# liyi14/mx-DeepIM

Hardware: NVIDIA H100
Metric: 480x640 4-iter pose refinements/sec (higher is better)
Workload: dtype fp16

## Files before the change

mx-deepim_b200/csrc/conv_igemm.cuh:

```cuda
#pragma once
#include <cuda.h>
#include <cuda_fp16.h>
#include "common.cuh"
#include "wgmma.cuh"

namespace dim {

struct ConvKParams {
  CUtensorMap a_map[4];
  CUtensorMap a_lo_map[4];
  CUtensorMap b_map;
  CUtensorMap b_lo_map;
  CUtensorMap out_map[2];
  const __nv_bfloat16 *in_hi, *in_lo;
  int in_cols;
  int KH, KW, stride, cchunks;
  int BW, BH, n_col_tiles;
  int Hq, Ho, Wo, Bn;
  int out_Hp, out_Wp, out_py, out_px, Cout;
  int kblocks;
  float slope;
  const float *bias;
  __nv_bfloat16 *out_hi, *out_lo;
  int in_off_r, in_off_c;
// ... 46 lines not shown
  do {
    asm volatile(
        "{\n\t.reg .pred p;\n\tmbarrier.try_wait.parity.shared::cta.b64 p, [%1], %2;\n\tselp.u32 %0, 1, 0, p;\n\t}"
        : "=r"(ok)
        : "r"(addr), "r"(parity)
        : "memory");
  } while (!ok);
}
__device__ __forceinline__ void prefetch_tmap(const CUtensorMap *m) {
  asm volatile("prefetch.tensormap [%0];" ::"l"((uint64_t)m) : "memory");
}
__device__ __forceinline__ void tma_load_2d(void *dst, const CUtensorMap *map, uint64_t *bar, int c0, int c1) {
  if (elect_one())
    asm volatile(
        "cp.async.bulk.tensor.2d.shared::cluster.global.mbarrier::complete_tx::bytes [%0], [%1, {%3, %4}], [%2];" ::"r"(
            smem_u32(dst)),
        "l"((uint64_t)map), "r"(smem_u32(bar)), "r"(c0), "r"(c1)
        : "memory");
}
__device__ __forceinline__ void tma_load_3d(void *dst, const CUtensorMap *map, uint64_t *bar, int c0, int c1, int c2) {
  if (elect_one())
    asm volatile(
        "cp.async.bulk.tensor.3d.shared::cluster.global.mbarrier::complete_tx::bytes [%0], [%1, {%3, %4, %5}], [%2];" ::
            "r"(smem_u32(dst)),
        "l"((uint64_t)map), "r"(smem_u32(bar)), "r"(c0), "r"(c1), "r"(c2)
        : "memory");
}

__device__ __forceinline__ void mbar_arrive(uint64_t *bar) {
  asm volatile("mbarrier.arrive.shared::cta.b64 _, [%0];" ::"r"(smem_u32(bar)) : "memory");
}

__device__ __forceinline__ void bulk_load_raw(void *dst, const void *src, uint32_t bytes, uint64_t *bar) {
  asm volatile("cp.async.bulk.shared::cluster.global.mbarrier::complete_tx::bytes [%0], [%1], %2, [%3];" ::"r"(smem_u32(dst)),
               "l"(src), "r"(bytes), "r"(smem_u32(bar))
               : "memory");
}
__device__ __forceinline__ void tma_store_4d(const CUtensorMap *map, const void *src, int c0, int c1, int c2, int c3) {
  asm volatile("cp.async.bulk.tensor.4d.global.shared::cta.bulk_group [%0, {%2, %3, %4, %5}], [%1];" ::"l"((uint64_t)map),
               "r"(smem_u32(src)), "r"(c0), "r"(c1), "r"(c2), "r"(c3)
               : "memory");
}
__device__ __forceinline__ void bulk_commit() { asm volatile("cp.async.bulk.commit_group;" ::: "memory"); }
__device__ __forceinline__ void bulk_wait_read0() { asm volatile("cp.async.bulk.wait_group.read 0;" ::: "memory"); }
__device__ __forceinline__ void bulk_wait0() { asm volatile("cp.async.bulk.wait_group 0;" ::: "memory"); }
__device__ __forceinline__ void named_bar_sync(int id, int threads) {
  asm volatile("bar.sync %0, %1;" ::"r"(id), "r"(threads) : "memory");
}
__device__ __forceinline__ void stmatrix_x4_trans(uint32_t addr, const uint32_t (&r)[4]) {
  asm volatile("stmatrix.sync.aligned.m8n8.x4.trans.shared.b16 [%0], {%1, %2, %3, %4};" ::"r"(addr), "r"(r[0]), "r"(r[1]),
               "r"(r[2]), "r"(r[3])
               : "memory");
}

__device__ __forceinline__ void tma_load_4d(void *dst, const CUtensorMap *map, uint64_t *bar, int c0, int c1, int c2, int c3) {
  if (elect_one())
    asm volatile(
        "cp.async.bulk.tensor.4d.shared::cluster.global.mbarrier::complete_tx::bytes [%0], [%1, {%3, %4, %5, %6}], [%2];" ::
            "r"(smem_u32(dst)),
        "l"((uint64_t)map), "r"(smem_u32(bar)), "r"(c0), "r"(c1), "r"(c2), "r"(c3)
        : "memory");
}

__device__ __forceinline__ uint64_t gmma_desc(uint32_t saddr, uint32_t lbo_bytes, uint32_t sbo_bytes, uint32_t layout) {
  uint64_t d = 0;
  d |= (uint64_t)((saddr & 0x3FFFFu) >> 4);
  d |= (uint64_t)((lbo_bytes >> 4) & 0x3FFFu) << 16;
  d |= (uint64_t)((sbo_bytes >> 4) & 0x3FFFu) << 32;
  d |= (uint64_t)layout << 62;
  return d;
}
constexpr uint32_t kSW128 = 1u, kSW64 = 2u, kNoSwizzle = 0u;

__device__ __forceinline__ void regs_producer() { asm volatile("setmaxnreg.dec.sync.aligned.u32 40;"); }
__device__ __forceinline__ void regs_consumer() { asm volatile("setmaxnreg.inc.sync.aligned.u32 232;"); }

}

__device__ __forceinline__ uint32_t pack2_f16(float a, float b) {
  uint32_t r;
  asm("cvt.rn.satfinite.f16x2.f32 %0, %1, %2;" : "=r"(r) : "f"(b), "f"(a));
  return r;
}
__device__ __forceinline__ uint32_t pack2_bf16(float a, float b) {
  uint32_t r;
  asm("cvt.rn.bf16x2.f32 %0, %1, %2;" : "=r"(r) : "f"(b), "f"(a));
  return r;
}

constexpr int kConv1Slack = 2048;


__device__ __forceinline__ int frag_row(int t) { return ((t >> 5) << 4) + ((t & 31) >> 2); }

__device__ __forceinline__ uint32_t pack2_bf16_lo(float v0, float v1, uint32_t hi) {
  return pack2_bf16(v0 - __uint_as_float(hi << 16), v1 - __uint_as_float(hi & 0xFFFF0000u));
}

template <bool SPLIT3, bool F16>
__device__ __forceinline__ void epi_pack(float v0, float v1, float b0, float b1, float slope, uint32_t &hi, uint32_t &lo) {
  v0 += b0;
  v1 += b1;
  v0 = v0 > 0.f ? v0 : v0 * slope;
  v1 = v1 > 0.f ? v1 : v1 * slope;
  if (F16) {
    hi = pack2_f16(v0, v1);
  } else {
    hi = pack2_bf16(v0, v1);
    if (SPLIT3) lo = pack2_bf16_lo(v0, v1, hi);
  }
}

template <bool SPLIT3, bool F16>
__device__ __forceinline__ void store_pair(float v0, float v1, float2 b, float slope, __nv_bfloat16 *out_hi, __nv_bfloat16 *out_lo,
                                           long long off) {
  uint32_t h, l = 0;
  epi_pack<SPLIT3, F16>(v0, v1, b.x, b.y, slope, h, l);
  *reinterpret_cast<uint32_t *>(out_hi + off) = h;
  if (SPLIT3) *reinterpret_cast<uint32_t *>(out_lo + off) = l;
}

template <bool SPLIT3>
__device__ __forceinline__ void store_pair_generic(float v0, float v1, const ConvKParams &p, int n, bool valid, long long off,
                                                   long long add_off, long long mask_off) {
  if (!valid || n >= p.Cout) return;
  if (p.bias) {
    v0 += __ldg(p.bias + n);
    v1 += __ldg(p.bias + n + 1);
  }
  if (p.addend.p) {
    const __nv_bfloat162 a = *reinterpret_cast<const __nv_bfloat162 *>(p.addend.p + add_off);
    if (SPLIT3) {
      const __nv_bfloat162 al = *reinterpret_cast<const __nv_bfloat162 *>(p.addend.lo + add_off);
      v0 += __low2float(a) + __low2float(al);
      v1 += __high2float(a) + __high2float(al);
    } else {
      v0 += __low2float(a);
      v1 += __high2float(a);
    }
  }
  if (p.mask.p) {
    if (n < p.mask_climit) {
      const __nv_bfloat162 m = *reinterpret_cast<const __nv_bfloat162 *>(p.mask.p + mask_off);
      if (!(__low2float(m) > 0.f)) v0 *= p.slope;
      if (!(__high2float(m) > 0.f)) v1 *= p.slope;
    }
  } else {
    v0 = v0 > 0.f ? v0 : v0 * p.slope;
    v1 = v1 > 0.f ? v1 : v1 * p.slope;
  }
  if (SPLIT3) {
    const uint32_t h = pack2_bf16(v0, v1);
    *reinterpret_cast<uint32_t *>(p.out_hi + off) = h;
    *reinterpret_cast<uint32_t *>(p.out_lo + off) = pack2_bf16_lo(v0, v1, h);
  } else {
    *reinterpret_cast<__nv_bfloat162 *>(p.out_hi + off) = __floats2bfloat162_rn(v0, v1);
  }
}

template <int BLOCK_N, int STAGES, bool SPLIT3>
struct ConvSmem2 {
  static constexpr int A_BYTES = 128 * 64 * 2;
  static constexpr int B_BYTES = BLOCK_N * 64 * 2;
  static constexpr int NPREC = SPLIT3 ? 2 : 1;
  static constexpr int STAGE_BYTES = (A_BYTES + B_BYTES) * NPREC;
  static constexpr int TOTAL = STAGES * STAGE_BYTES + 1024  + 256 ;
  static_assert(TOTAL <= 227 * 1024, "conv_igemm shared memory");
};

template <int BLOCK_N, int STAGES, bool SPLIT3, bool F16, int EPI = 0>
__global__ void __launch_bounds__(384, 1) conv_igemm_persistent_kernel(const __grid_constant__ ConvKParams p,
                                                                       const int total_tiles, const int n_tiles) {
  using S = ConvSmem2<BLOCK_N, STAGES, SPLIT3>;
  constexpr uint32_t SBO = 1024u;

  extern __shared__ uint8_t smem_raw[];
  uint8_t *smem = reinterpret_cast<uint8_t *>((reinterpret_cast<uintptr_t>(smem_raw) + 1023) & ~(uintptr_t)1023);
  uint64_t *full_bar = reinterpret_cast<uint64_t *>(smem + STAGES * S::STAGE_BYTES);
  uint64_t *empty_bar = full_bar + STAGES;

  const int wgi = threadIdx.x >> 7, warp = threadIdx.x >> 5;

  if (threadIdx.x == 0) {
    for (int s = 0; s < STAGES; ++s) {
      ptx::mbar_init(&full_bar[s], 1);
      ptx::mbar_init(&empty_bar[s], 2);
    }
    ptx::fence_barrier_init();
    ptx::prefetch_tmap(&p.b_map);
    ptx::prefetch_tmap(&p.a_map[0]);
  }
  __syncthreads();

  if (wgi == 0) {
    ptx::regs_producer();
    if (warp == 0) {
      const uint32_t tx = (uint32_t)(p.BW * p.BH * 64 * 2 + BLOCK_N * 64 * 2) * S::NPREC;
      int s = 0;
      uint32_t ph = 0;
      for (int tile = blockIdx.x; tile < total_tiles; tile += gridDim.x) {
        const int nt = tile % n_tiles, mt = tile / n_tiles;
        const int col_tile = mt % p.n_col_tiles, row_tile = mt / p.n_col_tiles;
        const int g0 = row_tile * p.BH, ow0 = col_tile * p.BW, n0 = nt * BLOCK_N;
        for (int kb = 0; kb < p.kblocks; ++kb) {
          ptx::mbar_wait(&empty_bar[s], ph ^ 1u);
          const int tap = kb / p.cchunks, cc = kb - tap * p.cchunks;
          const int kh = tap / p.KW, kw = tap - kh * p.KW;
          int view = 0, dr = kh, dc = kw;
          if (p.stride == 2) {
            view = ((kh & 1) << 1) | (kw & 1);
            dr = kh >> 1;
            dc = kw >> 1;
          }
          uint8_t *st = smem + s * S::STAGE_BYTES;
          if (EPI) { dr += p.in_off_r; dc += p.in_off_c; }
          if (ptx::elect_one()) {
            ptx::mbar_expect_tx_raw(&full_bar[s], tx);
            ptx::tma_load_3d_raw(st, &p.a_map[view], &full_bar[s], cc * 64, ow0 + dc, g0 + dr);
            ptx::tma_load_2d_raw(st + S::A_BYTES, &p.b_map, &full_bar[s], kb * 64, n0);
            if (SPLIT3) {
              ptx::tma_load_3d_raw(st + S::A_BYTES + S::B_BYTES, &p.a_lo_map[view], &full_bar[s], cc * 64, ow0 + dc, g0 + dr);
              ptx::tma_load_2d_raw(st + 2 * S::A_BYTES + S::B_BYTES, &p.b_lo_map, &full_bar[s], kb * 64, n0);
            }
          }
          __syncwarp();
          if (++s == STAGES) { s = 0; ph ^= 1u; }
        }
      }
    }
  } else {
    ptx::regs_consumer();
    const int t = threadIdx.x & 127;
    const int half = wgi - 1;
    const int r0 = half * 64 + frag_row(t), q2 = (t & 3) * 2;
    const bool arriver = t == 0;
    const uint32_t base = ptx::smem_u32(smem);
    float acc[BLOCK_N / 2];
    int s = 0;
    uint32_t ph = 0;
    for (int tile = blockIdx.x; tile < total_tiles; tile += gridDim.x) {
      int prev = -1;
      for (int kb = 0; kb < p.kblocks; ++kb) {
        ptx::mbar_wait(&full_bar[s], ph);
        const uint32_t a_hi = base + s * S::STAGE_BYTES + half * 8192;
        const uint32_t b_hi = base + s * S::STAGE_BYTES + S::A_BYTES;
        const uint64_t da0 = ptx::gmma_desc(a_hi, 16, SBO, ptx::kSW128), db0 = ptx::gmma_desc(b_hi, 16, SBO, ptx::kSW128);
        const uint64_t dal0 = da0 + ((S::A_BYTES + S::B_BYTES) >> 4), dbl0 = db0 + ((S::A_BYTES + S::B_BYTES) >> 4);
        wg::fence_acc(acc);
        wg::fence();
#pragma unroll
        for (int k = 0; k < 4; ++k) {
          const uint64_t da = da0 + (uint64_t)(2 * k), db = db0 + (uint64_t)(2 * k);
          wg::mma<BLOCK_N, F16, 0, 0>(acc, da, db, (kb > 0 || k > 0) ? 1u : 0u);
          if (SPLIT3) {
            wg::mma<BLOCK_N, false, 0, 0>(acc, dal0 + (uint64_t)(2 * k), db, 1u);
            wg::mma<BLOCK_N, false, 0, 0>(acc, da, dbl0 + (uint64_t)(2 * k), 1u);
          }
        }
        wg::commit();
        wg::wait<1>();
        wg::fence_acc(acc);
        if (prev >= 0 && arriver) ptx::mbar_arrive(&empty_bar[prev]);
        prev = s;
        if (++s == STAGES) { s = 0; ph ^= 1u; }
      }
      wg::wait<0>();
      wg::fence_acc(acc);
      if (prev >= 0 && arriver) ptx::mbar_arrive(&empty_bar[prev]);

      const int nt = tile % n_tiles, mt = tile / n_tiles;
      const int col_tile = mt % p.n_col_tiles, row_tile = mt / p.n_col_tiles;
      const int n0 = nt * BLOCK_N;
#pragma unroll
      for (int rr = 0; rr < 2; ++rr) {
        const int m = r0 + rr * 8;
        const int bh = m / p.BW, bw = m - bh * p.BW;
        const int g = row_tile * p.BH + bh, ow = col_tile * p.BW + bw;
        const int n_img = g / p.Hq, oh = g - n_img * p.Hq;
        if (EPI == 1) {
          const int y = oh * p.out_sy + p.out_oy, x = ow * p.out_sx + p.out_ox;
          const bool valid = (m < p.BW * p.BH) && (n_img < p.Bn) && (oh < p.Ho) && (ow < p.Wo) && y >= 0 && y < p.out_H &&
                             x >= 0 && x < p.out_W;
          const long long off =
              (((long long)n_img * p.out_Hp + y + p.out_py) * p.out_Wp + x + p.out_px) * p.out_cs + p.out_coff + n0 + q2;
          const long long add_off =
              (((long long)n_img * p.addend.Hp + y + p.addend.py) * p.addend.Wp + x + p.addend.px) * p.addend.cs + p.addend.coff +
              n0 + q2;
          const long long mask_off =
              (((long long)n_img * p.mask.Hp + y + p.mask.py) * p.mask.Wp + x + p.mask.px) * p.mask.cs + p.mask.coff + n0 + q2;
#pragma unroll
          for (int j = 0; j < BLOCK_N / 8; ++j)
            store_pair_generic<SPLIT3>(acc[4 * j + 2 * rr], acc[4 * j + 2 * rr + 1], p, n0 + 8 * j + q2, valid, off + 8 * j,
                               add_off + 8 * j, mask_off + 8 * j);
        } else {
          const bool valid = (m < p.BW * p.BH) && (n_img < p.Bn) && (oh < p.Ho) && (ow < p.Wo);
          if (valid) {
            const long long off = (((long long)n_img * p.out_Hp + oh + p.out_py) * p.out_Wp + ow + p.out_px) * p.Cout + n0 + q2;
#pragma unroll
            for (int j = 0; j < BLOCK_N / 8; ++j)
              store_pair<SPLIT3, F16>(acc[4 * j + 2 * rr], acc[4 * j + 2 * rr + 1],
                                      make_float2(__ldg(p.bias + n0 + 8 * j + q2), __ldg(p.bias + n0 + 8 * j + q2 + 1)), p.slope, p.out_hi,
                                      p.out_lo, off + 8 * j);
          }
        }
      }
    }
  }
}

constexpr int kConv1StoreN = 80;

template <int N, int STAGES, bool SPLIT3>
struct Conv1Smem {
  static constexpr int NPREC = SPLIT3 ? 2 : 1;
  static constexpr int TAP_BYTES = 64 * 32 * 2;
  static constexpr int RES_BYTES = 16 * TAP_BYTES * NPREC;
  static constexpr int STG_BYTES = N * 128;
  static constexpr int PLANE_BYTES = (N + 3) * 16;
  static constexpr int STRIP_BYTES = (4 * PLANE_BYTES + 127) / 128 * 128;
  static constexpr int STAGE_BYTES = STRIP_BYTES * NPREC;
  static constexpr int TOTAL = RES_BYTES + 2 * STG_BYTES * NPREC + STAGES * STAGE_BYTES + 1024  + 256 ;
  static_assert(N % kConv1StoreN == 0 && N % 16 == 0 && STG_BYTES % 1024 == 0, "conv1 tile width");
  static_assert(TOTAL <= 227 * 1024, "conv1 shared memory");
};

template <int N, int STAGES, bool SPLIT3, bool F16>
__global__ void __launch_bounds__(384, 1) conv1_kernel(const __grid_constant__ ConvKParams p, const int rows_total,
                                                       const int rows_per_chunk, const int chunks_per_col) {
  using S = Conv1Smem<N, STAGES, SPLIT3>;
  extern __shared__ uint8_t smem_raw[];
  uint8_t *smem = reinterpret_cast<uint8_t *>((reinterpret_cast<uintptr_t>(smem_raw) + 1023) & ~(uintptr_t)1023);
  uint8_t *res = smem;
  uint8_t *stg = res + S::RES_BYTES;
  uint8_t *ring = stg + 2 * S::NPREC * S::STG_BYTES;
  uint64_t *full_bar = reinterpret_cast<uint64_t *>(ring + STAGES * S::STAGE_BYTES);
  uint64_t *empty_bar = full_bar + STAGES;
  uint64_t *res_bar = empty_bar + STAGES;

  const int wgi = threadIdx.x >> 7, warp = threadIdx.x >> 5;
  const int ct = blockIdx.x / chunks_per_col, ck = blockIdx.x - ct * chunks_per_col;
  const int g_lo = ck * rows_per_chunk;
  const int g_hi = min(rows_total, g_lo + rows_per_chunk);
  const int n_rows = max(0, g_hi - g_lo);
  const int n_strips = n_rows > 0 ? n_rows + 3 : 0;
  const int ow0 = ct * N;

  if (threadIdx.x == 0) {
    for (int s = 0; s < STAGES; ++s) {
      ptx::mbar_init(&full_bar[s], 1);
      ptx::mbar_init(&empty_bar[s], 2);
    }
    ptx::mbar_init(res_bar, 1);
    ptx::fence_barrier_init();
    ptx::prefetch_tmap(&p.b_map);
    ptx::prefetch_tmap(&p.out_map[0]);
  }
  __syncthreads();

  if (wgi == 0) {
// ... 260 lines not shown
```

mx-deepim_b200/csrc/net.cu:

```cuda
#include <cuda_fp16.h>
#include <string.h>

#include <memory>
#include <mutex>

#include "launch.cuh"
#include "net_state.cuh"

namespace dim {

static void build_geometry(NetState *ns, int H, int W) {
  int h = H, w = W;
  for (int i = 0; i < 10; ++i) {
    const LayerSpec &s = kLayers[i];
    LayerGeom &g = ns->g[i];
    g.Cin = s.Cin; g.Cout = s.Cout; g.k = s.k; g.stride = s.stride; g.pad = s.pad;
    g.Hin = h; g.Win = w;
    g.Ho = (h + 2 * s.pad - s.k) / s.stride + 1;
    g.Wo = (w + 2 * s.pad - s.k) / s.stride + 1;
    if (g.Ho < 1) g.Ho = 1;
    if (g.Wo < 1) g.Wo = 1;
    int Hp = h + 2 * s.pad, Wp = w + 2 * s.pad;
    if (s.stride == 2) { Hp += Hp & 1; Wp += Wp & 1; }
    g.py = g.px = s.pad;
// ... 26 lines not shown
    if (i == 0) {
      const int nt = cdiv(g.Wo, 128);
      g.BW = cdiv(g.Wo, nt); g.BH = 1; g.n_col_tiles = nt;
    }
    g.kblocks = g.KH * g.KW * (g.Ceff / g.BLOCK_K);
    h = g.Ho; w = g.Wo;
  }
}

typedef CUresult (*EncodeTiledFn)(CUtensorMap *, CUtensorMapDataType, cuuint32_t, void *, const cuuint64_t *,
                                  const cuuint64_t *, const cuuint32_t *, const cuuint32_t *, CUtensorMapInterleave,
                                  CUtensorMapSwizzle, CUtensorMapL2promotion, CUtensorMapFloatOOBfill);
static EncodeTiledFn get_encode() {
  static EncodeTiledFn fn = nullptr;
  if (!fn) {
    void *p = nullptr;
    cudaDriverEntryPointQueryResult q;
    if (cudaGetDriverEntryPoint("cuTensorMapEncodeTiled", &p, cudaEnableDefault, &q) == cudaSuccess &&
        q == cudaDriverEntryPointSuccess)
      fn = reinterpret_cast<EncodeTiledFn>(p);
  }
  return fn;
}

int encode_map(CUtensorMap *m, void *base, int rank, const uint64_t *dims, const uint64_t *strides_bytes,
                      const uint32_t *box, int block_k ) {
  EncodeTiledFn fn = get_encode();
  DIM_REQUIRE(fn != nullptr, "cuTensorMapEncodeTiled entry point not available (driver too old?)");
  cuuint64_t gd[5]; cuuint64_t gs[5]; cuuint32_t bx[5]; cuuint32_t es[5];
  for (int i = 0; i < rank; ++i) { gd[i] = dims[i]; bx[i] = box[i]; es[i] = 1; }
  for (int i = 0; i < rank - 1; ++i) gs[i] = strides_bytes[i];
  CUresult r = fn(m, CU_TENSOR_MAP_DATA_TYPE_BFLOAT16, (cuuint32_t)rank, base, gd, gs, bx, es,
                  CU_TENSOR_MAP_INTERLEAVE_NONE,
                  block_k == 64 ? CU_TENSOR_MAP_SWIZZLE_128B
                                : (block_k == 32 ? CU_TENSOR_MAP_SWIZZLE_64B : CU_TENSOR_MAP_SWIZZLE_NONE),
                  CU_TENSOR_MAP_L2_PROMOTION_L2_256B, CU_TENSOR_MAP_FLOAT_OOB_FILL_NONE);
  if (r != CUDA_SUCCESS) {
    set_error("cuTensorMapEncodeTiled failed with CUresult %d (rank %d dims %llu %llu %llu box %u %u %u)", (int)r, rank,
              (unsigned long long)dims[0], (unsigned long long)dims[1], (unsigned long long)(rank > 2 ? dims[2] : 0),
              box[0], box[1], rank > 2 ? box[2] : 0);
    return 3;
  }
  return 0;
}

static int build_maps(NetState *ns, int B, bool f16, TensorMaps &tm) {
  for (int i = 0; i < 10; ++i) {
    const LayerGeom &g = ns->g[i];
    ConvKParams &kp = tm.kp[i];
    memset(&kp, 0, sizeof(kp));
    for (int lo = 0; lo < 2; ++lo) {
      __nv_bfloat16 *base = lo ? ns->act_lo[i] : ns->act_hi[i];
      CUtensorMap *maps = lo ? kp.a_lo_map : kp.a_map;
      const uint32_t box[3] = {(uint32_t)g.BLOCK_K, (uint32_t)g.BW, (uint32_t)g.BH};
      if (i == 0 && ns->input_depth) {
        const uint64_t dims[4] = {8, (uint64_t)g.cols, 8, (uint64_t)B * g.rows};
        const uint64_t str[3] = {16, (uint64_t)g.cols * 16, (uint64_t)g.cols * 128};
        const uint32_t box4[4] = {8, (uint32_t)(g.BW + 3), 8, 1};
        if (int rc = encode_map(&maps[0], base, 4, dims, str, box4, 0)) return rc;
        maps[1] = maps[2] = maps[3] = maps[0];
      } else if (i == 0) {
      } else if (g.stride_eff == 1) {
        const uint64_t dims[3] = {(uint64_t)g.Cbuf, (uint64_t)g.cols, (uint64_t)B * g.rows};
        const uint64_t str[2] = {(uint64_t)g.Cbuf * 2, (uint64_t)g.cols * g.Cbuf * 2};
        if (int rc = encode_map(&maps[0], base, 3, dims, str, box, g.BLOCK_K)) return rc;
        maps[1] = maps[2] = maps[3] = maps[0];
      } else {
        for (int ph = 0; ph < 2; ++ph)
          for (int pw = 0; pw < 2; ++pw) {
            const uint64_t dims[3] = {(uint64_t)g.Cbuf, (uint64_t)g.cols / 2, (uint64_t)B * g.rows / 2};
            const uint64_t str[2] = {(uint64_t)2 * g.Cbuf * 2, (uint64_t)2 * g.cols * g.Cbuf * 2};
            __nv_bfloat16 *vb = base + ((size_t)ph * g.cols + pw) * g.Cbuf;
            if (int rc = encode_map(&maps[(ph << 1) | pw], vb, 3, dims, str, box, g.BLOCK_K)) return rc;
          }
      }
    }
    {
      const uint64_t Ktot = (uint64_t)g.KH * g.KW * g.Ceff;
      const uint64_t dims[2] = {Ktot, (uint64_t)g.Cout};
      const uint64_t str[1] = {Ktot * 2};
      const uint32_t box[2] = {(uint32_t)g.BLOCK_K, (uint32_t)(i == 0 && ns->input_depth ? 16 : g.BLOCK_N)};
      __nv_bfloat16 *wop = f16 ? ns->w_f16[i] : ns->w_hi[i];
      if (int rc = encode_map(&kp.b_map, wop, 2, dims, str, box, g.BLOCK_K)) return rc;
      if (int rc = encode_map(&kp.b_lo_map, ns->w_lo[i], 2, dims, str, box, g.BLOCK_K)) return rc;
    }
    kp.KH = g.KH; kp.KW = g.KW; kp.stride = g.stride_eff; kp.cchunks = g.Ceff / g.BLOCK_K;
    kp.BW = g.BW; kp.BH = g.BH; kp.n_col_tiles = g.n_col_tiles;
    kp.Hq = g.Hq; kp.Ho = g.Ho; kp.Wo = g.Wo; kp.Bn = B;
    if (i < 9) {
      const LayerGeom &nx = ns->g[i + 1];
      kp.out_Hp = nx.rows; kp.out_Wp = nx.cols; kp.out_py = nx.py; kp.out_px = nx.px;
    } else {
      kp.out_Hp = g.Ho; kp.out_Wp = g.Wo; kp.out_py = 0; kp.out_px = 0;
    }
    kp.Cout = g.Cout;
    kp.kblocks = g.kblocks;
    kp.slope = 0.1f;
    kp.bias = ns->bias[i];
    kp.out_hi = ns->act_hi[i + 1];
    kp.out_lo = ns->act_lo[i + 1];
    if (i == 0 && !ns->input_depth) {
      const LayerGeom &nx = ns->g[1];
      kp.in_hi = ns->act_hi[0];
      kp.in_lo = ns->act_lo[0];
      kp.in_cols = g.cols;
      const uint64_t dims[4] = {64, (uint64_t)g.Wo, (uint64_t)g.Ho, (uint64_t)B};
      const uint64_t str[3] = {128, (uint64_t)nx.cols * 128, (uint64_t)nx.rows * nx.cols * 128};
      const uint32_t box[4] = {64, (uint32_t)kConv1StoreN, 1, 1};
      const size_t interior = ((size_t)nx.py * nx.cols + nx.px) * 64;
      for (int lo = 0; lo < 2; ++lo)
        if (int rc = encode_map(&kp.out_map[lo], (lo ? ns->act_lo[1] : ns->act_hi[1]) + interior, 4, dims, str, box, 64)) return rc;
    }
  }
  return 0;
}

template <bool F16>
__device__ __forceinline__ void mma_bf16_16816(float *c, const uint32_t *a, uint32_t b0, uint32_t b1) {
  if (F16)
    asm volatile(
        "mma.sync.aligned.m16n8k16.row.col.f32.f16.f16.f32 {%0,%1,%2,%3}, {%4,%5,%6,%7}, {%8,%9}, {%0,%1,%2,%3};"
        : "+f"(c[0]), "+f"(c[1]), "+f"(c[2]), "+f"(c[3])
        : "r"(a[0]), "r"(a[1]), "r"(a[2]), "r"(a[3]), "r"(b0), "r"(b1));
  else
    asm volatile(
        "mma.sync.aligned.m16n8k16.row.col.f32.bf16.bf16.f32 {%0,%1,%2,%3}, {%4,%5,%6,%7}, {%8,%9}, {%0,%1,%2,%3};"
        : "+f"(c[0]), "+f"(c[1]), "+f"(c[2]), "+f"(c[3])
        : "r"(a[0]), "r"(a[1]), "r"(a[2]), "r"(a[3]), "r"(b0), "r"(b1));
}

template <bool S3, bool F16 = false>
__global__ void __launch_bounds__(256) fc6_mma_kernel(const __nv_bfloat16 *__restrict__ act_hi,
                                                      const __nv_bfloat16 *__restrict__ act_lo,
                                                      const __nv_bfloat16 *__restrict__ w_hi,
                                                      const __nv_bfloat16 *__restrict__ w_lo, int B, int max_batch,
                                                      float *__restrict__ partial) {
  constexpr int PITCH = FC6_KC * 2 + 64;
  __shared__ __align__(16) uint8_t a_hi_s[16 * PITCH];
  __shared__ __align__(16) uint8_t a_lo_s[S3 ? 16 * PITCH : 16];
  const int s = blockIdx.x, k0 = s * FC6_KC;
  const int warp = threadIdx.x >> 5, lane = threadIdx.x & 31, g = lane >> 2, q = lane & 3;
  for (int b0 = 0; b0 < B; b0 += 16) {
    const int nb = min(16, B - b0);
    __syncthreads();
    for (int idx = threadIdx.x; idx < 16 * (FC6_KC / 8); idx += blockDim.x) {
      const int r = idx / (FC6_KC / 8), c8 = idx - r * (FC6_KC / 8);
      uint4 vh = make_uint4(0, 0, 0, 0), vl = make_uint4(0, 0, 0, 0);
      if (r < nb) {
        const size_t o = (size_t)(b0 + r) * FC6_K + k0 + c8 * 8;
        vh = *reinterpret_cast<const uint4 *>(act_hi + o);
        if (S3) vl = *reinterpret_cast<const uint4 *>(act_lo + o);
      }
      *reinterpret_cast<uint4 *>(a_hi_s + r * PITCH + c8 * 16) = vh;
      if (S3) *reinterpret_cast<uint4 *>(a_lo_s + r * PITCH + c8 * 16) = vl;
    }
    __syncthreads();
    float acc[4][4];
#pragma unroll
    for (int t = 0; t < 4; ++t)
#pragma unroll
      for (int e = 0; e < 4; ++e) acc[t][e] = 0.f;
#pragma unroll 2
    for (int kc = 0; kc < FC6_KC; kc += 32) {
      const uint4 ah0 = *reinterpret_cast<const uint4 *>(a_hi_s + g * PITCH + (kc + q * 8) * 2);
// ... 232 lines not shown
  ns->f16_stale = false;
  return 0;
}

int net_load(dim_ctx *ctx, const float *const *W, const float *const *Bv) {
  NetState *ns = ctx->net;
  DIM_REQUIRE(ns != nullptr, "net not created");
  DIM_REQUIRE(ns->net_ok, "dim_net_load: FlowNetS + fc6 (81920 inputs) needs a 480x640 context");
  DIM_REQUIRE(!ns->train_aliased, "dim_net_load: this context trains; use dim_train_load_params (it owns the weights)");
  if (ns->loaded) DIM_CHECK(cudaDeviceSynchronize());
  if (int rc = net_alloc_weights(ctx)) return rc;
  size_t n[12], off[13] = {0};
  for (int i = 0; i < 10; ++i) {
    const LayerGeom &g = ns->g[i];
    const int cin = i == 0 && !ns->input_depth ? (ns->input_mask ? 8 : 6) : g.Cin;
    n[i] = (size_t)g.Cout * cin * g.k * g.k;
  }
  n[10] = (size_t)256 * FC6_K;
  n[11] = 256 * 256;
  for (int i = 0; i < 12; ++i) off[i + 1] = off[i] + n[i];
  float *stage_p = nullptr;
  DIM_CHECK(cudaMalloc(&stage_p, off[12] * sizeof(float)));
  std::unique_ptr<float, cudaError_t (*)(void *)> stage(stage_p, cudaFree);
  auto put = [](float *dst, const float *src, size_t count) {
    return cudaMemcpy(dst, src, count * sizeof(float), cudaMemcpyHostToDevice);
  };
  const float *w[12];
  for (int i = 0; i < 12; ++i) {
    w[i] = stage.get() + off[i];
    if (i != 10) DIM_CHECK(put(stage.get() + off[i], W[i], n[i]));
  }
  {
    std::vector<float> p((size_t)256 * FC6_K);
    for (int o = 0; o < 256; ++o)
      for (int c = 0; c < 1024; ++c)
        for (int hw = 0; hw < 80; ++hw) p[(size_t)o * FC6_K + (size_t)hw * 1024 + c] = W[10][(size_t)o * FC6_K + (size_t)c * 80 + hw];
    DIM_CHECK(put(stage.get() + off[10], p.data(), n[10]));
  }
  for (int i = 0; i < 10; ++i) DIM_CHECK(put(ns->bias[i], Bv[i], ns->g[i].Cout));
  DIM_CHECK(put(ns->fc6_b, Bv[10], 256));
  DIM_CHECK(put(ns->fc7_b, Bv[11], 256));
  DIM_CHECK(put(ns->rot_w, W[12], 4 * 256));
  DIM_CHECK(put(ns->rot_b, Bv[12], 4));
  DIM_CHECK(put(ns->trans_w, W[13], 3 * 256));
  DIM_CHECK(put(ns->trans_b, Bv[13], 3));
  if (int rc = net_pack_weights(ctx, w, 0, true, true)) return rc;
  DIM_CHECK(cudaStreamSynchronize(0));
  ns->loaded = true;
  return 0;
}

template <int BN, int ST, bool S3, bool F16>
static int launch_conv(const ConvKParams &kp, int total_tiles, int n_tiles, int cap, cudaStream_t st) {
  using S = ConvSmem2<BN, ST, S3>;
  static bool attr_set = false;
  if (!attr_set) {
    DIM_CHECK(cudaFuncSetAttribute(conv_igemm_persistent_kernel<BN, ST, S3, F16>, cudaFuncAttributeMaxDynamicSharedMemorySize,
                                   S::TOTAL));
    attr_set = true;
  }
  const int grid = total_tiles < cap ? total_tiles : cap;
  conv_igemm_persistent_kernel<BN, ST, S3, F16><<<grid, 384, S::TOTAL, st>>>(kp, total_tiles, n_tiles);
  DIM_LAUNCH_CHECK();
  return 0;
}

template <int N, int ST, bool S3, bool F16>
static int launch_conv1(const ConvKParams &kp, int grid, int rows_total, int rpc, int chunks, cudaStream_t st) {
  using S = Conv1Smem<N, ST, S3>;
  static bool set = false;
  if (!set) {
    DIM_CHECK(cudaFuncSetAttribute(conv1_kernel<N, ST, S3, F16>, cudaFuncAttributeMaxDynamicSharedMemorySize, S::TOTAL));
    set = true;
  }
  conv1_kernel<N, ST, S3, F16><<<grid, 384, S::TOTAL, st>>>(kp, rows_total, rpc, chunks);
  DIM_LAUNCH_CHECK();
  return 0;
}

template <int ST, bool S3, bool F16, int NB>
static int launch_conv1_rgbd(const ConvKParams &kp, int grid, int rows_total, int rpc, int chunks, int strip_bytes,
                             cudaStream_t st) {
  const int smem_bytes = 16 * NB * 128 * (S3 ? 2 : 1) + ST * (S3 ? 2 : 1) * strip_bytes + kConv1Slack + 1024 + 256;
  DIM_REQUIRE(smem_bytes <= 227 * 1024, "conv1 (RGB-D): image too wide for the rolling-strip ring");
  static int set = 0;
  if (set < smem_bytes) {
    DIM_CHECK(cudaFuncSetAttribute(conv1_rgbd_kernel<ST, S3, F16, NB>, cudaFuncAttributeMaxDynamicSharedMemorySize,
                                   smem_bytes));
    set = smem_bytes;
  }
  conv1_rgbd_kernel<ST, S3, F16, NB><<<grid, 384, smem_bytes, st>>>(kp, rows_total, rpc, chunks, strip_bytes);
  DIM_LAUNCH_CHECK();
  return 0;
}

int net_set_input_depth(dim_ctx *ctx, bool enable) {
  NetState *ns = ctx->net;
  DIM_REQUIRE(ns != nullptr, "net not created");
  if (ns->input_depth == enable) return 0;
  DIM_REQUIRE(!ns->loaded, "dim_ctx_set_input_depth: call it before dim_net_load (this context's weights are loaded)");
  if (!ns->act0_rgb_hi) { ns->act0_rgb_hi = ns->act_hi[0]; ns->act0_rgb_lo = ns->act_lo[0]; }
  ns->input_depth = enable;
  build_geometry(ns, ctx->H, ctx->W);
  ns->maps.clear();
  const LayerGeom &g = ns->g[0];
  const size_t per = (size_t)g.rows * g.cols * g.Cbuf;
  ns->act_elems_per_image[0] = per;
// ... 162 lines not shown
```

mx-deepim_b200/csrc/train.cu:

```cuda
#include <string.h>

#include <algorithm>

#include "conv_wgrad.cuh"
#include "launch.cuh"
#include "net_state.cuh"

namespace dim {

enum { PK_CONV = 0, PK_FC = 1, PK_DECONV = 2, PK_FROZEN = 3 };
struct ParamSpec {
  const char *name;
  int kind, d0, d1, k;
};
static const ParamSpec kParams[24] = {
    {"flow_conv1", PK_CONV, 64, 8, 7},   {"conv2", PK_CONV, 128, 64, 5},    {"conv3", PK_CONV, 256, 128, 5},
    {"conv3_1", PK_CONV, 256, 256, 3},   {"conv4", PK_CONV, 512, 256, 3},   {"conv4_1", PK_CONV, 512, 512, 3},
    {"conv5", PK_CONV, 512, 512, 3},     {"conv5_1", PK_CONV, 512, 512, 3}, {"conv6", PK_CONV, 1024, 512, 3},
    {"conv6_1", PK_CONV, 1024, 1024, 3}, {"fc6", PK_FC, 256, 81920, 1},     {"fc7", PK_FC, 256, 256, 1},
    {"rot", PK_FC, 4, 256, 1},           {"trans", PK_FC, 3, 256, 1},
    {"Convolution1", PK_CONV, 2, 1024, 3}, {"deconv5", PK_DECONV, 1024, 512, 4}, {"upsample_flow6to5", PK_DECONV, 2, 2, 4},
    {"Convolution2", PK_CONV, 2, 1026, 3}, {"deconv4", PK_DECONV, 1026, 256, 4}, {"upsample_flow5to4", PK_DECONV, 2, 2, 4},
    {"Convolution3", PK_CONV, 2, 770, 3},  {"mask_conv3", PK_CONV, 1, 770, 3},
    {"upsampling", PK_FROZEN, 2, 1, 32},   {"mask_upsampling", PK_FROZEN, 1, 1, 32}};
// ... 846 lines not shown
  const bool s3 = precision == DIM_PREC_BF16X3;
  if (s3 == ts->s3) return 0;
  if (s3) {
    DIM_CHECK(cudaDeviceSynchronize());
    if (!ts->lo_alloc)
      if (int rc = alloc_lo(ctx, ts)) return rc;
    if (ctx->net->loaded && ctx->net->train_aliased) {
      if (int rc = repack_all(ctx, ts->side[3], true)) return rc;
      DIM_CHECK(cudaStreamSynchronize(ts->side[3]));
    }
  }
  ts->s3 = s3;
  return 0;
}

int train_get_precision(dim_ctx *ctx, int *precision) {
  TrainState *ts = train_of(ctx);
  DIM_REQUIRE(ts != nullptr, "dim_train_get_precision: call dim_train_create first");
  *precision = ts->s3 ? DIM_PREC_BF16X3 : DIM_PREC_BF16;
  return 0;
}

int train_get_params(dim_ctx *ctx, float *flat_host, size_t n, int which, cudaStream_t st) {
  TrainState *ts = train_of(ctx);
  DIM_REQUIRE(ts != nullptr && n == ts->n_params, "dim_train_get_params: bad state or size");
  DIM_CHECK(cudaMemcpyAsync(flat_host, which ? ts->mom : ts->master, n * sizeof(float), cudaMemcpyDeviceToHost, st));
  DIM_CHECK(cudaStreamSynchronize(st));
  return 0;
}

size_t train_param_count(dim_ctx *ctx) { TrainState *ts = train_of(ctx); return ts ? ts->n_params : 0; }
int train_param_info(int idx, const char **name, long long *w_numel, long long *b_numel, bool input_depth, bool input_mask) {
  if (idx < 0 || idx >= 24) return 1;
  const ParamSpec s = param_spec(idx, input_depth, input_mask);
  *name = s.name; *w_numel = (long long)param_numel(s); *b_numel = (long long)bias_numel(s);
  return 0;
}

static void pick_tile(int W, int rows_total, int cap, int &BW, int &BH, int max_bw = 1 << 30, int max_bh = 1 << 30) {
  for (int pass = 0; pass < 2; ++pass) {
    long best = -1;
    for (int bw = 1; bw <= cap; bw <<= 1) {
      const int bh = cap / bw;
      if (pass == 0 && (bw > max_bw || bh > max_bh)) continue;
      const long cost = (long)cdiv(W, bw) * bw * cdiv(rows_total, bh) * bh;
      if (best < 0 || cost < best || (cost == best && bw > BW)) { best = cost; BW = bw; BH = bh; }
    }
    if (best >= 0) return;
  }
}

template <int BN, int ST, bool S3 = false>
static int launch_generic(const ConvKParams &kp, int total_tiles, int n_tiles, int cap, cudaStream_t st) {
  using S = ConvSmem2<BN, ST, S3>;
  static bool attr_set = false;
  if (!attr_set) {
    DIM_CHECK(cudaFuncSetAttribute(conv_igemm_persistent_kernel<BN, ST, S3, false, 1>,
                                   cudaFuncAttributeMaxDynamicSharedMemorySize, S::TOTAL));
    attr_set = true;
  }
  const int grid = total_tiles < cap ? total_tiles : cap;
  conv_igemm_persistent_kernel<BN, ST, S3, false, 1><<<grid, 384, S::TOTAL, st>>>(kp, total_tiles, n_tiles);
  DIM_LAUNCH_CHECK();
  return 0;
}

static int run_generic(dim_ctx *ctx, const ConvKParams &kp, const LayerGeom &g, int B, cudaStream_t st, bool s3) {
  const int n_tiles = cdiv(g.Cout, g.BLOCK_N);
  const int total = cdiv(B * g.Hq, g.BH) * g.n_col_tiles * n_tiles;
  const int sms = ctx->num_sms;
  if (s3) {
    if (g.BLOCK_N == 256) return launch_generic<256, 2, true>(kp, total, n_tiles, sms, st);
    if (g.BLOCK_N == 128) return launch_generic<128, 3, true>(kp, total, n_tiles, sms, st);
    return launch_generic<64, 4, true>(kp, total, n_tiles, sms, st);
  }
  if (g.BLOCK_N == 256) return launch_generic<256, 4>(kp, total, n_tiles, sms, st);
  if (g.BLOCK_N == 128) return launch_generic<128, 6>(kp, total, n_tiles, sms, st);
  return launch_generic<64, 8>(kp, total, n_tiles, sms, st);
}

static int make_generic(ConvKParams &kp, LayerGeom &g, int B, const Buf &in, int in_coff, int K_ch, bool stride2, int KH, int KW,
                        int off_r, int off_c, int Ho, int Wo, const __nv_bfloat16 *w, const __nv_bfloat16 *w_lo, int N,
                        const float *bias, float slope, const Buf &out, int out_coff, int sy, int sx, int oy, int ox,
                        const Buf *addend, int add_coff, const Buf *mask, int mask_coff, int mask_climit, bool s3) {
  memset(&kp, 0, sizeof(kp));
  memset(&g, 0, sizeof(g));
  g.Cout = N; g.KH = KH; g.KW = KW; g.BLOCK_K = 64;
  g.BLOCK_N = (N % 256 == 0) ? 256 : ((N % 128 == 0) ? 128 : 64);
  g.Hq = stride2 ? in.Hp / 2 : in.Hp;
  pick_tile(Wo, B * g.Hq, 128, g.BW, g.BH, stride2 ? in.Wp / 2 : in.Wp, B * g.Hq);
  g.n_col_tiles = cdiv(Wo, g.BW);
  g.kblocks = KH * KW * (K_ch / 64);
  const uint32_t box[3] = {64u, (uint32_t)g.BW, (uint32_t)g.BH};
  for (int lo = 0; lo < (s3 ? 2 : 1); ++lo) {
    __nv_bfloat16 *base = lo ? in.lo : in.p;
    CUtensorMap *a_map = lo ? kp.a_lo_map : kp.a_map;
    if (!stride2) {
      const uint64_t dims[3] = {(uint64_t)K_ch, (uint64_t)in.Wp, (uint64_t)B * in.Hp};
      const uint64_t str[2] = {(uint64_t)in.C * 2, (uint64_t)in.Wp * in.C * 2};
      if (int rc = encode_map(&a_map[0], base + in_coff, 3, dims, str, box, 64)) return rc;
      a_map[1] = a_map[2] = a_map[3] = a_map[0];
    } else {
      for (int ph = 0; ph < 2; ++ph)
        for (int pw = 0; pw < 2; ++pw) {
          const uint64_t dims[3] = {(uint64_t)K_ch, (uint64_t)in.Wp / 2, (uint64_t)B * in.Hp / 2};
          const uint64_t str[2] = {(uint64_t)2 * in.C * 2, (uint64_t)2 * in.Wp * in.C * 2};
          if (int rc = encode_map(&a_map[(ph << 1) | pw], base + ((size_t)ph * in.Wp + pw) * in.C + in_coff, 3, dims, str, box, 64))
// ... 553 lines not shown
```

Before: 3159.

## Stage conv epilogue through shared memory with stmatrix and TMA bulk stores

Result: faster. 3324, median of 6 (+5.2%).

```diff
diff --git a/mx-deepim_b200/csrc/conv_igemm.cuh b/mx-deepim_b200/csrc/conv_igemm.cuh
--- a/mx-deepim_b200/csrc/conv_igemm.cuh
+++ b/mx-deepim_b200/csrc/conv_igemm.cuh
@@ -122,6 +122,11 @@
                "r"(r[2]), "r"(r[3])
                : "memory");
 }
+__device__ __forceinline__ void stmatrix_x4(uint32_t addr, const uint32_t (&r)[4]) {
+  asm volatile("stmatrix.sync.aligned.m8n8.x4.shared.b16 [%0], {%1, %2, %3, %4};" ::"r"(addr), "r"(r[0]), "r"(r[1]), "r"(r[2]),
+               "r"(r[3])
+               : "memory");
+}
 
 __device__ __forceinline__ void tma_load_4d(void *dst, const CUtensorMap *map, uint64_t *bar, int c0, int c1, int c2, int c3) {
   if (elect_one())
@@ -228,25 +233,33 @@
   }
 }
 
-template <int BLOCK_N, int STAGES, bool SPLIT3>
+template <int BLOCK_N, int STAGES, bool SPLIT3, int EPI>
 struct ConvSmem2 {
   static constexpr int A_BYTES = 128 * 64 * 2;
   static constexpr int B_BYTES = BLOCK_N * 64 * 2;
   static constexpr int NPREC = SPLIT3 ? 2 : 1;
   static constexpr int STAGE_BYTES = (A_BYTES + B_BYTES) * NPREC;
-  static constexpr int TOTAL = STAGES * STAGE_BYTES + 1024  + 256 ;
-  static_assert(TOTAL <= 227 * 1024, "conv_igemm shared memory");
+  static constexpr int RING_BYTES = STAGES * STAGE_BYTES;
+  static constexpr int LIMIT = 227 * 1024, FIXED = 1024  + 256 ;
+  static constexpr bool TMA_EPI = EPI == 0 && !SPLIT3;
+  static constexpr int STG_GROUPS =
+      !TMA_EPI ? 0 : (RING_BYTES + 2 * BLOCK_N * 128 + FIXED <= LIMIT ? BLOCK_N / 64 : BLOCK_N / 128);
+  static constexpr int STG_ROUNDS = TMA_EPI ? BLOCK_N / 64 / STG_GROUPS : 0;
+  static constexpr int STG_BYTES = STG_GROUPS * 8192;
+  static constexpr int TOTAL = RING_BYTES + 2 * STG_BYTES + FIXED;
+  static_assert(TOTAL <= LIMIT, "conv_igemm shared memory");
 };
 
 template <int BLOCK_N, int STAGES, bool SPLIT3, bool F16, int EPI = 0>
 __global__ void __launch_bounds__(384, 1) conv_igemm_persistent_kernel(const __grid_constant__ ConvKParams p,
                                                                        const int total_tiles, const int n_tiles) {
-  using S = ConvSmem2<BLOCK_N, STAGES, SPLIT3>;
+  using S = ConvSmem2<BLOCK_N, STAGES, SPLIT3, EPI>;
   constexpr uint32_t SBO = 1024u;
 
   extern __shared__ uint8_t smem_raw[];
   uint8_t *smem = reinterpret_cast<uint8_t *>((reinterpret_cast<uintptr_t>(smem_raw) + 1023) & ~(uintptr_t)1023);
-  uint64_t *full_bar = reinterpret_cast<uint64_t *>(smem + STAGES * S::STAGE_BYTES);
+  uint8_t *stg = smem + S::RING_BYTES;
+  uint64_t *full_bar = reinterpret_cast<uint64_t *>(stg + 2 * S::STG_BYTES);
   uint64_t *empty_bar = full_bar + STAGES;
 
   const int wgi = threadIdx.x >> 7, warp = threadIdx.x >> 5;
@@ -259,6 +272,7 @@
     ptx::fence_barrier_init();
     ptx::prefetch_tmap(&p.b_map);
     ptx::prefetch_tmap(&p.a_map[0]);
+    if (S::TMA_EPI) ptx::prefetch_tmap(&p.out_map[0]);
   }
   __syncthreads();
 
@@ -286,11 +300,12 @@
           if (EPI) { dr += p.in_off_r; dc += p.in_off_c; }
           if (ptx::elect_one()) {
             ptx::mbar_expect_tx_raw(&full_bar[s], tx);
-            ptx::tma_load_3d_raw(st, &p.a_map[view], &full_bar[s], cc * 64, ow0 + dc, g0 + dr);
-            ptx::tma_load_2d_raw(st + S::A_BYTES, &p.b_map, &full_bar[s], kb * 64, n0);
-            if (SPLIT3) {
-              ptx::tma_load_3d_raw(st + S::A_BYTES + S::B_BYTES, &p.a_lo_map[view], &full_bar[s], cc * 64, ow0 + dc, g0 + dr);
-              ptx::tma_load_2d_raw(st + 2 * S::A_BYTES + S::B_BYTES, &p.b_lo_map, &full_bar[s], kb * 64, n0);
+            for (int pr = 0; pr < S::NPREC; ++pr) {
+              uint8_t *sa = st + pr * (S::A_BYTES + S::B_BYTES);
+              const CUtensorMap *am = pr ? &p.a_lo_map[view] : &p.a_map[view];
+              ptx::tma_load_3d_raw(sa, am, &full_bar[s], cc * 64, ow0 + dc, g0 + dr);
+              if (EPI == 0) ptx::tma_load_3d_raw(sa + S::A_BYTES / 2, am, &full_bar[s], cc * 64, ow0 + dc, g0 + dr + (p.BH >> 1));
+              ptx::tma_load_2d_raw(sa + S::A_BYTES, pr ? &p.b_lo_map : &p.b_map, &full_bar[s], kb * 64, n0);
             }
           }
           __syncwarp();
@@ -302,9 +317,13 @@
     ptx::regs_consumer();
     const int t = threadIdx.x & 127;
     const int half = wgi - 1;
-    const int r0 = half * 64 + frag_row(t), q2 = (t & 3) * 2;
+    const int q2 = (t & 3) * 2;
     const bool arriver = t == 0;
     const uint32_t base = ptx::smem_u32(smem);
+    uint8_t *my_stg = stg + half * S::STG_BYTES;
+    const int lane = t & 31;
+    const uint32_t st_addr = ptx::smem_u32(my_stg) + (uint32_t)((16 * (t >> 5) + 8 * ((lane >> 3) & 1) + (lane & 7)) * 128);
+    const uint32_t st_sw = (uint32_t)(((lane >> 4) & 1) ^ (lane & 7));
     float acc[BLOCK_N / 2];
     int s = 0;
     uint32_t ph = 0;
@@ -341,40 +360,88 @@
       const int nt = tile % n_tiles, mt = tile / n_tiles;
       const int col_tile = mt % p.n_col_tiles, row_tile = mt / p.n_col_tiles;
       const int n0 = nt * BLOCK_N;
-#pragma unroll
-      for (int rr = 0; rr < 2; ++rr) {
-        const int m = r0 + rr * 8;
-        const int bh = m / p.BW, bw = m - bh * p.BW;
-        const int g = row_tile * p.BH + bh, ow = col_tile * p.BW + bw;
-        const int n_img = g / p.Hq, oh = g - n_img * p.Hq;
-        if (EPI == 1) {
-          const int y = oh * p.out_sy + p.out_oy, x = ow * p.out_sx + p.out_ox;
-          const bool valid = (m < p.BW * p.BH) && (n_img < p.Bn) && (oh < p.Ho) && (ow < p.Wo) && y >= 0 && y < p.out_H &&
-                             x >= 0 && x < p.out_W;
-          const long long off =
-              (((long long)n_img * p.out_Hp + y + p.out_py) * p.out_Wp + x + p.out_px) * p.out_cs + p.out_coff + n0 + q2;
-          const long long add_off =
-              (((long long)n_img * p.addend.Hp + y + p.addend.py) * p.addend.Wp + x + p.addend.px) * p.addend.cs + p.addend.coff +
-              n0 + q2;
-          const long long mask_off =
-              (((long long)n_img * p.mask.Hp + y + p.mask.py) * p.mask.Wp + x + p.mask.px) * p.mask.cs + p.mask.coff + n0 + q2;
-#pragma unroll
-          for (int j = 0; j < BLOCK_N / 8; ++j)
-            store_pair_generic<SPLIT3>(acc[4 * j + 2 * rr], acc[4 * j + 2 * rr + 1], p, n0 + 8 * j + q2, valid, off + 8 * j,
-                               add_off + 8 * j, mask_off + 8 * j);
-        } else {
-          const bool valid = (m < p.BW * p.BH) && (n_img < p.Bn) && (oh < p.Ho) && (ow < p.Wo);
-          if (valid) {
-            const long long off = (((long long)n_img * p.out_Hp + oh + p.out_py) * p.out_Wp + ow + p.out_px) * p.Cout + n0 + q2;
+      if constexpr (S::TMA_EPI) {
+        const int gs = row_tile * p.BH + half * (p.BH >> 1), ow0 = col_tile * p.BW;
+        const int n_img = gs / p.Hq, oh = gs - n_img * p.Hq;
+        const bool store0 = n_img < p.Bn && oh < p.Ho, store1 = n_img + 1 < p.Bn && oh + (p.BH >> 1) > p.Hq;
+#pragma unroll
+        for (int rd = 0; rd < S::STG_ROUNDS; ++rd) {
+          if (arriver) ptx::bulk_wait_read0();
+          ptx::named_bar_sync(1 + half, 128);
+#pragma unroll
+          for (int i = 0; i < S::STG_GROUPS * 4; ++i) {
+            const int j = rd * S::STG_GROUPS * 8 + 2 * i;
+            const float *bj = p.bias + n0 + 8 * j + q2;
+            const float b0 = __ldg(bj), b1 = __ldg(bj + 1), b2 = __ldg(bj + 8), b3 = __ldg(bj + 9);
+            uint32_t h[4], unused;
+            epi_pack<false, F16>(acc[4 * j + 0], acc[4 * j + 1], b0, b1, p.slope, h[0], unused);
+            epi_pack<false, F16>(acc[4 * j + 2], acc[4 * j + 3], b0, b1, p.slope, h[1], unused);
+            epi_pack<false, F16>(acc[4 * j + 4], acc[4 * j + 5], b2, b3, p.slope, h[2], unused);
+            epi_pack<false, F16>(acc[4 * j + 6], acc[4 * j + 7], b2, b3, p.slope, h[3], unused);
+            ptx::stmatrix_x4(st_addr + (uint32_t)((i >> 2) * 8192) + (((uint32_t)(2 * (i & 3)) ^ st_sw) << 4), h);
+          }
+          ptx::fence_proxy_async();
+          ptx::named_bar_sync(1 + half, 128);
+          if (arriver && store0) {
+            for (int q = 0; q < S::STG_GROUPS; ++q)
+              ptx::tma_store_4d(&p.out_map[0], my_stg + q * 8192, n0 + (rd * S::STG_GROUPS + q) * 64, ow0, oh, n_img);
+            ptx::bulk_commit();
+          }
+        }
+        if (store1) {
+#pragma unroll
+          for (int rr = 0; rr < 2; ++rr) {
+            const int lr = frag_row(t) + rr * 8, bh = lr / p.BW;
+            const int oh1 = oh + bh - p.Hq, ow = ow0 + lr - bh * p.BW;
+            if (lr < p.BW * (p.BH >> 1) && oh1 >= 0 && oh1 < p.Ho) {
+              const long long off =
+                  (((long long)(n_img + 1) * p.out_Hp + oh1 + p.out_py) * p.out_Wp + ow + p.out_px) * p.Cout + n0 + q2;
+#pragma unroll
+              for (int j = 0; j < BLOCK_N / 8; ++j)
+                store_pair<false, F16>(acc[4 * j + 2 * rr], acc[4 * j + 2 * rr + 1],
+                                       make_float2(__ldg(p.bias + n0 + 8 * j + q2), __ldg(p.bias + n0 + 8 * j + q2 + 1)), p.slope,
+                                       p.out_hi, p.out_lo, off + 8 * j);
+            }
+          }
+        }
+      } else {
+#pragma unroll
+        for (int rr = 0; rr < 2; ++rr) {
+          const int lr = frag_row(t) + rr * 8, m = EPI ? half * 64 + lr : lr;
+          const bool in_tile = EPI ? m < p.BW * p.BH : lr < p.BW * (p.BH >> 1);
+          const int bh = m / p.BW, bw = m - bh * p.BW;
+          const int g = row_tile * p.BH + (EPI ? 0 : half * (p.BH >> 1)) + bh, ow = col_tile * p.BW + bw;
+          const int n_img = g / p.Hq, oh = g - n_img * p.Hq;
+          if (EPI == 1) {
+            const int y = oh * p.out_sy + p.out_oy, x = ow * p.out_sx + p.out_ox;
+            const bool valid = in_tile && (n_img < p.Bn) && (oh < p.Ho) && (ow < p.Wo) && y >= 0 && y < p.out_H &&
+                               x >= 0 && x < p.out_W;
+            const long long off =
+                (((long long)n_img * p.out_Hp + y + p.out_py) * p.out_Wp + x + p.out_px) * p.out_cs + p.out_coff + n0 + q2;
+            const long long add_off =
+                (((long long)n_img * p.addend.Hp + y + p.addend.py) * p.addend.Wp + x + p.addend.px) * p.addend.cs + p.addend.coff +
+                n0 + q2;
+            const long long mask_off =
+                (((long long)n_img * p.mask.Hp + y + p.mask.py) * p.mask.Wp + x + p.mask.px) * p.mask.cs + p.mask.coff + n0 + q2;
 #pragma unroll
             for (int j = 0; j < BLOCK_N / 8; ++j)
-              store_pair<SPLIT3, F16>(acc[4 * j + 2 * rr], acc[4 * j + 2 * rr + 1],
-                                      make_float2(__ldg(p.bias + n0 + 8 * j + q2), __ldg(p.bias + n0 + 8 * j + q2 + 1)), p.slope, p.out_hi,
-                                      p.out_lo, off + 8 * j);
-          }
-        }
-      }
-    }
+              store_pair_generic<SPLIT3>(acc[4 * j + 2 * rr], acc[4 * j + 2 * rr + 1], p, n0 + 8 * j + q2, valid, off + 8 * j,
+                                 add_off + 8 * j, mask_off + 8 * j);
+          } else {
+            const bool valid = in_tile && (n_img < p.Bn) && (oh < p.Ho) && (ow < p.Wo);
+            if (valid) {
+              const long long off = (((long long)n_img * p.out_Hp + oh + p.out_py) * p.out_Wp + ow + p.out_px) * p.Cout + n0 + q2;
+#pragma unroll
+              for (int j = 0; j < BLOCK_N / 8; ++j)
+                store_pair<SPLIT3, F16>(acc[4 * j + 2 * rr], acc[4 * j + 2 * rr + 1],
+                                        make_float2(__ldg(p.bias + n0 + 8 * j + q2), __ldg(p.bias + n0 + 8 * j + q2 + 1)), p.slope, p.out_hi,
+                                        p.out_lo, off + 8 * j);
+            }
+          }
+        }
+      }
+    }
+    if (S::TMA_EPI && arriver) ptx::bulk_wait0();
   }
 }
 
diff --git a/mx-deepim_b200/csrc/net.cu b/mx-deepim_b200/csrc/net.cu
--- a/mx-deepim_b200/csrc/net.cu
+++ b/mx-deepim_b200/csrc/net.cu
@@ -102,7 +102,7 @@
     for (int lo = 0; lo < 2; ++lo) {
       __nv_bfloat16 *base = lo ? ns->act_lo[i] : ns->act_hi[i];
       CUtensorMap *maps = lo ? kp.a_lo_map : kp.a_map;
-      const uint32_t box[3] = {(uint32_t)g.BLOCK_K, (uint32_t)g.BW, (uint32_t)g.BH};
+      const uint32_t box[3] = {(uint32_t)g.BLOCK_K, (uint32_t)g.BW, (uint32_t)(g.BH / 2)};
       if (i == 0 && ns->input_depth) {
         const uint64_t dims[4] = {8, (uint64_t)g.cols, 8, (uint64_t)B * g.rows};
         const uint64_t str[3] = {16, (uint64_t)g.cols * 16, (uint64_t)g.cols * 128};
@@ -150,16 +150,21 @@
     kp.out_hi = ns->act_hi[i + 1];
     kp.out_lo = ns->act_lo[i + 1];
     if (i == 0 && !ns->input_depth) {
-      const LayerGeom &nx = ns->g[1];
       kp.in_hi = ns->act_hi[0];
       kp.in_lo = ns->act_lo[0];
       kp.in_cols = g.cols;
-      const uint64_t dims[4] = {64, (uint64_t)g.Wo, (uint64_t)g.Ho, (uint64_t)B};
-      const uint64_t str[3] = {128, (uint64_t)nx.cols * 128, (uint64_t)nx.rows * nx.cols * 128};
-      const uint32_t box[4] = {64, (uint32_t)kConv1StoreN, 1, 1};
-      const size_t interior = ((size_t)nx.py * nx.cols + nx.px) * 64;
-      for (int lo = 0; lo < 2; ++lo)
-        if (int rc = encode_map(&kp.out_map[lo], (lo ? ns->act_lo[1] : ns->act_hi[1]) + interior, 4, dims, str, box, 64)) return rc;
+    }
+    if (i > 0 || !ns->input_depth) {
+      DIM_REQUIRE(i == 0 || (g.BH % 2 == 0 && g.BH / 2 <= g.Hq && g.BW * (g.BH / 2) <= 64),
+                  "conv_igemm: a consumer warpgroup's box must be whole output rows within two images");
+      const uint64_t cb = (uint64_t)g.Cout * 2;
+      const uint64_t dims[4] = {(uint64_t)g.Cout, (uint64_t)g.Wo, (uint64_t)g.Ho, (uint64_t)B};
+      const uint64_t str[3] = {cb, (uint64_t)kp.out_Wp * cb, (uint64_t)kp.out_Hp * kp.out_Wp * cb};
+      const uint32_t box[4] = {64, (uint32_t)(i == 0 ? kConv1StoreN : g.BW), (uint32_t)(i == 0 ? 1 : g.BH / 2), 1};
+      const size_t interior = ((size_t)kp.out_py * kp.out_Wp + kp.out_px) * g.Cout;
+      for (int lo = 0; lo < (i == 0 ? 2 : 1); ++lo)
+        if (int rc = encode_map(&kp.out_map[lo], (lo ? ns->act_lo[i + 1] : ns->act_hi[i + 1]) + interior, 4, dims, str, box, 64))
+          return rc;
     }
   }
   return 0;
@@ -498,7 +503,7 @@
 
 template <int BN, int ST, bool S3, bool F16>
 static int launch_conv(const ConvKParams &kp, int total_tiles, int n_tiles, int cap, cudaStream_t st) {
-  using S = ConvSmem2<BN, ST, S3>;
+  using S = ConvSmem2<BN, ST, S3, 0>;
   static bool attr_set = false;
   if (!attr_set) {
     DIM_CHECK(cudaFuncSetAttribute(conv_igemm_persistent_kernel<BN, ST, S3, F16>, cudaFuncAttributeMaxDynamicSharedMemorySize,
diff --git a/mx-deepim_b200/csrc/train.cu b/mx-deepim_b200/csrc/train.cu
--- a/mx-deepim_b200/csrc/train.cu
+++ b/mx-deepim_b200/csrc/train.cu
@@ -922,7 +922,7 @@
 
 template <int BN, int ST, bool S3 = false>
 static int launch_generic(const ConvKParams &kp, int total_tiles, int n_tiles, int cap, cudaStream_t st) {
-  using S = ConvSmem2<BN, ST, S3>;
+  using S = ConvSmem2<BN, ST, S3, 1>;
   static bool attr_set = false;
   if (!attr_set) {
     DIM_CHECK(cudaFuncSetAttribute(conv_igemm_persistent_kernel<BN, ST, S3, false, 1>,
```
